# lks1248/SPH-EXA

Hardware: AMD Instinct MI355X
Metric: particle-updates/sec (whole node), Sedov -n 400, 1/2/4/8 MI355X + HBM roofline % (higher is better)
Workload: dtype f32 hydro / f64 coordinates (sph::SphTypes)

## Files before the change

sph-exa_amd/csrc/sx_sim.hpp:

```cpp
#pragma once

#include <hip/hip_runtime.h>

#include <cmath>
#include <initializer_list>
#include <string>
#include <utility>
#include <vector>

#include "../../include/sphexa_hip.h"
#include "sx_comm.hpp"
#include "sx_hydro.hpp"
#include "sx_map.hpp"
#include "sx_profile.hpp"
#include "sx_fof.hpp"
#include "sx_twopoint.hpp"
#include "sx_spectrum.hpp"
#include "sx_step_timer.hpp"
#include "sx_tree.hpp"

namespace sx::turb
{
struct SimTurb;
}
// ... 61 lines not shown
    int      cleanSinceBuild{0};
    uint64_t plainSteps{0};
    uint64_t builds{0}, reuseSteps{0}, staleClusters{0}, exactClusters{0};
    uint64_t resyncs{0};
    uint32_t lastStale{0}, lastExact{0};
    uint64_t stepClusters{0}, stepS13{0};
    bool      xmFused{false};
    uint32_t* exactList{nullptr};
    bool      listsKept{false};
    const void *keptNloc{nullptr}, *keptUni{nullptr}, *keptMask{nullptr}, *keptSame{nullptr}, *keptFrz{nullptr},
        *keptNlocB{nullptr};
    uint64_t  keptClusters{0}, frozenClusters{0};
    uint64_t  earlyExact{0};
    sx::ListsB lb{};
};


struct SkinBuffers
{
    float *   dx{nullptr}, *dy{nullptr}, *dz{nullptr};
    uint32_t* cells{nullptr};
    float *   rel{nullptr}, *hb{nullptr}, *acc{nullptr};
    uint32_t *sloc{nullptr}, *scnt{nullptr}, *ucountS{nullptr}, *l1{nullptr}, *l2{nullptr}, *l3{nullptr};
    uint32_t* host{nullptr};
    uint8_t * streak{nullptr}, *same{nullptr};
    uint32_t* hitmask{nullptr};
    float2*   frz{nullptr};
    uint32_t *nlocB{nullptr}, *ucountB{nullptr}, *hitmaskB{nullptr};
    double *drift{nullptr}, *relg{nullptr}, *x0{nullptr}, *y0{nullptr}, *z0{nullptr};
    float* h0{nullptr};
};

struct ReqBox;

struct DomBuffers
{
    uint32_t* bins{nullptr};
    uint64_t *split{nullptr}, *seg{nullptr}, *cnth{nullptr};
    uint32_t *agree{nullptr}, *agreeh{nullptr};
    unsigned *hflag{nullptr}, *hflagh{nullptr};
    uint32_t* errh{nullptr};
    ReqBox*   mybox{nullptr};
};

struct GravBuffers
{
// ... 135 lines not shown
```

sph-exa_amd/csrc/sx_sim_skin.cpp:

```cpp
#include "sx_sim_internal.hpp"

using namespace sx;
using namespace sx::sim;

namespace
{

__global__ void coverListKernel(const uint32_t* list, uint32_t maxList, uint32_t first, uint32_t last, const double* x,
                                const double* y, const double* z, const float* r, float scale, const ReqBox* boxes,
                                DevBox box, double qmargin, const double* drift, const double* x0, const double* y0,
                                const double* z0, const double* relg, unsigned* flag)
{
    const uint32_t k = blockIdx.x;
    if (k >= min(list[0], maxList)) return;
    const uint32_t i = first + list[1 + k] * kCluster + threadIdx.x;
    if (i >= last) return;
    const ReqBox& b  = boxes[(i - first) / kChunk];
    const double  R  = 2.0 * (double)r[i] * (double)scale * (1.0 + 1e-6) + qmargin;
    const double  Ra = R + drift[0], Rr = R + relg[i];
    const bool    outNow = fabs(foldPbc(x[i] - b.c[0], box, 0)) + Ra > b.s[0] ||
                        fabs(foldPbc(y[i] - b.c[1], box, 1)) + Ra > b.s[1] ||
                        fabs(foldPbc(z[i] - b.c[2], box, 2)) + Ra > b.s[2];
    const bool    outBuild = fabs(foldPbc(x0[i] - b.c[0], box, 0)) + Rr > b.s[0] ||
                          fabs(foldPbc(y0[i] - b.c[1], box, 1)) + Rr > b.s[1] ||
// ... 113 lines not shown
    const bool   ok = skinReserveDisp(s);
    const auto&  B  = s->skinBuf;
    q.dispX = B.dx, q.dispY = B.dy, q.dispZ = B.dz, q.cells = B.cells;
    q.grid  = skinGrid(s->dbox);
    if (!ok) return false;
    return hipMemsetAsync(q.cells, 0xff, 3 * nc * sizeof(uint32_t), st) == hipSuccess &&
           hipMemsetAsync(q.cells + 3 * nc, 0, 3 * nc * sizeof(uint32_t), st) == hipSuccess;
}

static bool skinReserveSearch(sx_sim* s, const NsArgs& na, uint32_t ncl, bool twoSets)
{
    auto&      B    = s->skinBuf;
    auto&      M    = s->mem;
    const bool disp = skinReserveDisp(s);
    B.rel     = M.get<float>("skin.rel", s->cap);
    B.sloc    = M.get<uint32_t>("skin.sloc", na.numGroups * (size_t)nlocWords(s->skin.ngmaxS) * kWave);
    B.scnt    = M.get<uint32_t>("skin.scnt", s->cap);
    B.hb      = M.get<float>("skin.hb", s->cap);
    B.acc     = M.get<float>("skin.acc", ncl);
    B.ucountS = M.get<uint32_t>("skin.ucount", ncl);
    B.l1      = M.get<uint32_t>("skin.l1", ncl + 1);
    B.l2      = M.get<uint32_t>("skin.l2", ncl + 1);
    B.l3      = M.get<uint32_t>("skin.l3", ncl + 1);
    B.host    = M.pinned<uint32_t>("skin.host", 4);
    B.streak  = M.get<uint8_t>("skin.streak", ncl);
    B.hitmask = M.get<uint32_t>("skin.hitmask", na.numGroups * (size_t)kSkinMaskWords * kWave);
    B.same    = M.get<uint8_t>("skin.same", ncl);
    B.frz     = M.get<float2>("skin.frz", ncl);
    B.nlocB    = twoSets ? M.get<uint32_t>("skin.nlocB", na.numGroups * (size_t)nlocWords(na.ngmax) * kWave) : nullptr;
    B.ucountB  = twoSets ? M.get<uint32_t>("skin.ucountB", ncl) : nullptr;
    B.hitmaskB = twoSets ? M.get<uint32_t>("skin.hitmaskB", na.numGroups * (size_t)kSkinMaskWords * kWave) : nullptr;
    return disp && B.rel && B.sloc && B.scnt && B.hb && B.acc && B.ucountS && B.l1 && B.l2 && B.l3 && B.host &&
           B.streak && B.hitmask && B.same && B.frz && (!twoSets || (B.nlocB && B.ucountB && B.hitmaskB));
}

int skinSearch(sx_sim* s, const NsArgs& na, bool reuse, hipStream_t st, float* xmOut, RecT* rtXm, SkinCounts& out)
{
    auto&          K   = s->skin;
    const uint32_t ncl = (na.numGroups + kClusterWaves - 1) / kClusterWaves;
    out                = SkinCounts{};
    out.clusters       = ncl;
    if (!reuse) K.built = K.cur;
    if (!ncl) return SX_OK;
    if (!reuse) K.ngmaxS = skinCapacity(s->p.ngmax, K.built);
    const bool twoSets = na.ucap / 4 >= (uint32_t)kSkinCap && !getenv("SX_SKIN_ONESET");
    if (!skinReserveSearch(s, na, ncl, twoSets)) return SX_ERR_NOMEM;
    const SkinBuffers& B = s->skinBuf;
    uint32_t *const l1 = B.l1, *const l2 = B.l2, *const l3 = B.l3, *const hl = B.host;
    uint32_t* const hmask = B.hitmask, *const nlocB = B.nlocB;
    uint8_t* const  same  = B.same;
    float2* const   frz   = B.frz;

    const SkinGrid g = skinGrid(s->dbox);
    SkinArgs fa{};
    fa.first = na.first, fa.last = na.last, fa.numGroups = na.numGroups, fa.ngmax = na.ngmax, fa.ng0 = na.ng0;
// ... 20 lines not shown
    b.skin1    = 1.0f + K.built;
    b.iterateH = 0;
    b.nloc     = B.sloc;
    b.packMax  = 0;
    b.ngmax    = K.ngmaxS;
    b.nc       = B.scnt;
    b.rxOut    = nullptr;
    b.uoff     = uoff;
    b.ucount   = B.ucountS;

    SIM_HIP(hipMemsetAsync(l1, 0, 4, st));
    SIM_HIP(hipMemsetAsync(l2, 0, 4, st));
    if (!reuse)
    {
        SIM_HIP(hipMemsetAsync(B.streak, 0, ncl, st));
        SIM_HIP(findNeighbors(b, st));
        fa.fresh = 1;
    }
    else fa.fresh = 0;
    fa.list  = nullptr;
    fa.stale = l1;
    fa.streak = reuse ? B.streak : nullptr;
    fa.direct = reuse ? l2 : nullptr;
    SIM_HIP(skinFilter(fa, ncl, st));
    SIM_HIP(hipMemcpyAsync(hl, l1, 4, hipMemcpyDeviceToHost, st));
    SIM_HIP(hipMemcpyAsync(hl + 1, l2, 4, hipMemcpyDeviceToHost, st));
    SIM_HIP(hipStreamSynchronize(st));
    const uint32_t n1 = hl[0], nd = hl[1];
    uint32_t       n2 = nd;
    out.rebuilt = n1, out.stale = n1 + nd, out.exact = nd;
    NsArgs         x  = na;
    NsPolicy large;
    large.mode = 1;
    if (reuse) b.policy = x.policy = &large;
    if ((n1 || nd) && reuse)
    {
        double* c3 = s->mem.get<double>("skin.centers", 3 * (size_t)s->tree.numNodes);
        double* s3 = s->mem.get<double>("skin.sizes", 3 * (size_t)s->tree.numNodes);
        if (!c3 || !s3) return SX_ERR_NOMEM;
        SIM_HIP(skinRefreshBoxes(s->tree, na.x, na.y, na.z, na.box, c3, s3, st));
        b.centers = x.centers = c3;
        b.sizes = x.sizes = s3;
    }
    const bool early = n1 && nd && reuse && s->auxStream && s->evAuxIn && s->evAuxOut && !getenv("SX_SKIN_SERIAL_EXACT");
    if (early)
    {
// ... 6 lines not shown
        if (!sh || atoi(sh) != 0)
        {
            const unsigned G = searchGrid();
            xd.maxGrid       = std::min(nd, G / 2);
            b.maxGrid        = G - xd.maxGrid;
        }
        if (!xd.work || !xd.hSave || !xd.hitMasks) return SX_ERR_NOMEM;
        SIM_HIP(hipEventRecord(s->evAuxIn, st));
        SIM_HIP(hipStreamWaitEvent(s->auxStream, s->evAuxIn, 0));
        SIM_HIP(findNeighbors(xd, s->auxStream));
        SIM_HIP(hipEventRecord(s->evAuxOut, s->auxStream));
    }
    uint32_t* lx = l2;
    if (n1)
    {
        b.subset  = l1;
        SIM_HIP(findNeighbors(b, st));
        fa.fresh  = 1;
        fa.list   = l1;
        if (early) SIM_HIP(hipMemsetAsync(l3, 0, 4, st));
        fa.stale  = early ? l3 : l2;
        fa.streak = nullptr;
        fa.direct = nullptr;
        SIM_HIP(skinFilter(fa, ncl, st));
        SIM_HIP(hipMemcpyAsync(hl + 2, fa.stale, 4, hipMemcpyDeviceToHost, st));
        SIM_HIP(hipStreamSynchronize(st));
        n2 = hl[2];
    }
    uint32_t n3 = 0;
    if (early)
    {
        n3 = n2, n2 = nd + n3, lx = l3;
        K.earlyExact += nd;
        SIM_HIP(hipStreamWaitEvent(st, s->evAuxOut, 0));
    }
    out.exact = n2;
    {
        if (early ? n3 : n2)
        {
            x.subset = lx;
            SIM_HIP(findNeighbors(x, st));
        }
        if (early)
        {
            if (n3) SIM_HIP(hipMemcpyAsync(l2 + 1 + nd, l3 + 1, 4 * (size_t)n3, hipMemcpyDeviceToDevice, st));
            hl[3] = n2;
// ... 121 lines not shown
```

sph-exa_amd/csrc/sx_skin.hip:

```cpp
#include "sx_kernel_poly.hpp"
#include "sx_skin.hpp"
#include "sx_traverse.hpp"

namespace sx
{

namespace
{

constexpr int kWalkPF  = 8;
constexpr int kWalkBlocks = (nlocWords(256) + kWalkPF - 1) / kWalkPF;
constexpr int kB       = kCluster;

__device__ __forceinline__ int cellIndex(double v, const SkinGrid& g, int d) { return gridCell(v, g, d); }

__device__ __forceinline__ float keepOrZero(float v, bool k)
{
    return __builtin_bit_cast(float, __builtin_bit_cast(uint32_t, v) & (0u - (uint32_t)k));
}

__device__ __forceinline__ float norm3up(float x, float y, float z)
{
    return sqrtf(fmaf(x, x, fmaf(y, y, z * z))) * (1.0f + 0x1p-18f) + 1e-30f;
}
// ... 95 lines not shown
    {
        for (int k = 1; k < (int)(blockDim.x >> 6); ++k)
            mx = max(mx, s_max[0][k]), mu = max(mu, s_max[1][k]), kp += s_max[2][k], fz += s_max[3][k], st += s_sum[0][k],
            te += s_sum[1][k], un += s_sum[2][k];
        stats[2]                                          = mx;
        stats[18]                                         = kp;
        stats[19]                                         = fz;
        stats[12]                                         = mu;
        *reinterpret_cast<unsigned long long*>(stats + 4) = st;
        *reinterpret_cast<unsigned long long*>(stats + 6) = te;
        *reinterpret_cast<unsigned long long*>(stats + 8) = un;
    }
}

__device__ __forceinline__ void pushStale(const SkinArgs& a, uint32_t c)
{
    uint32_t* L = (a.direct && a.streak && a.streak[c]) ? a.direct : a.stale;
    L[1 + atomicAdd(&L[0], 1u)] = c;
    if (a.streak) a.streak[c] = 1;
    if (a.same) a.same[c] = 0;
}
static_assert((kWalkBlocks + 1) / 2 <= (int)kSkinMaskWords, "hit-mask words per target");

__global__ __launch_bounds__(kB) __attribute__((amdgpu_waves_per_eu(4))) void skinFilterKernel(SkinArgs a,
                                                                                              uint32_t numClusters)
{
    __shared__ float4   s_rec[kSkinCap];
    __shared__ uint8_t  s_hit[kSkinCap + 4];
    __shared__ uint16_t s_bm[kWalkBlocks][kB];
    uint16_t* const     s_rank = reinterpret_cast<uint16_t*>(s_rec);
    __shared__ float    s_red[kClusterWaves];
    __shared__ int      s_vote[kClusterWaves];
    __shared__ uint32_t s_wsum[kClusterWaves];
    __shared__ uint4    s_cst[kClusterWaves];

    const uint32_t nWork = a.list ? __builtin_amdgcn_readfirstlane(a.list[0]) : numClusters;
    if (blockIdx.x >= nWork) return;
    const uint32_t blk  = a.list ? blockIdx.x : xcdBlock(blockIdx.x, gridDim.x);
    const uint32_t c    = __builtin_amdgcn_readfirstlane(a.list ? a.list[1 + blk] : blk);
    const int      wave = __builtin_amdgcn_readfirstlane(threadIdx.x >> 6), lane = threadIdx.x & 63;
    const uint32_t gw   = c * kClusterWaves + wave;
    const uint32_t c0   = a.first + c * kCluster;
    const uint32_t i    = c0 + threadIdx.x;
    const bool     valid = gw < a.numGroups && i < a.last;
    const uint32_t iS    = valid ? i : c0;
    const double   xi = a.x[iS], yi = a.y[iS], zi = a.z[iS];
    const double   ox = a.x[c0], oy = a.y[c0], oz = a.z[c0];
    float          hi   = a.h[iS];
    const float    h0   = hi;
    const float    hbi  = a.fresh ? hi : a.hb[iS];
    const float    ux = a.dispX[c0], uy = a.dispY[c0], uz = a.dispZ[c0];
    const float    di = a.fresh ? 0.0f
                                : a.rel[iS] + norm3up(a.dispX[iS] - ux, a.dispY[iS] - uy, a.dispZ[iS] - uz);
    const float    Ri = 2.0f * (hbi * a.skin1);
    const uint32_t scount = valid ? a.scnt[i] - 1u : 0u;
    const uint32_t U      = __builtin_amdgcn_readfirstlane(a.ucountS[c]);
    const float    kEps   = 0x1p-16f;
    const uint32_t lstate    = (a.same && a.keepLists && !a.fresh) ? (uint32_t)a.same[c] : 0u;
    const uint32_t lcur      = (a.nlocB && (lstate & kListsBSel)) ? 1u : 0u;
    const bool     curValid  = ((lstate >> lcur) & 1u) != 0;
    const bool     mayFreeze = a.frz && curValid;
    const float2   fref      = mayFreeze ? a.frz[c] : make_float2(-INFINITY, -INFINITY);
    auto           blockBits = [&](uint32_t v) -> uint32_t {
        uint32_t w = 0;
#pragma unroll
        for (int k = 0; k < 3; ++k)
            w |= __ballot((v >> k) & 1u) != 0 ? 1u << k : 0u;
        if (lane == 0) s_vote[wave] = (int)w;
        __syncthreads();
        uint32_t any = 0;
        for (int k = 0; k < kClusterWaves; ++k)
            any |= (uint32_t)s_vote[k];
        __syncthreads();
        return any;
    };
    auto blockAny = [&](bool v) -> bool { return blockBits(v ? 1u : 0u) != 0; };

    float A = 0.0f;
    if (!a.fresh)
    {
        const double rx = foldPbc(xi - ox, a.box, 0), ry = foldPbc(yi - oy, a.box, 1), rz = foldPbc(zi - oz, a.box, 2);
        double       lo[3]  = {valid ? rx : INFINITY, valid ? ry : INFINITY, valid ? rz : INFINITY};
        double       hb3[3] = {valid ? rx : -INFINITY, valid ? ry : -INFINITY, valid ? rz : -INFINITY};
        float        rmax   = valid ? Ri : 0.0f;
        for (int d = 0; d < 3; ++d)
        {
            lo[d]  = -waveMax(-lo[d]);
            hb3[d] = waveMax(hb3[d]);
        }
        rmax      = waveMax(rmax);
        float gmx = 0.0f;
        if (rmax > 0.0f)
        {
            const double o[3] = {ox, oy, oz};
            int          k0[3], nk[3];
            uint32_t     total = 1;
            for (int d = 0; d < 3; ++d)
            {
                k0[d]  = cellIndex(o[d] + lo[d] - (double)rmax, a.grid, d);
                int k1 = cellIndex(o[d] + hb3[d] + (double)rmax, a.grid, d);
                nk[d]  = k1 - k0[d] + 1;
                if (a.grid.pbc[d] && nk[d] >= a.grid.n) k0[d] = 0, nk[d] = a.grid.n;
                total *= nk[d];
            }
            for (uint32_t q = lane; q < total; q += kWave)
            {
                int      k[3];
                uint32_t r = q;
                for (int d = 0; d < 3; ++d)
                {
                    const uint32_t rq = r / (uint32_t)nk[d];
                    k[d]              = k0[d] + (int)(r - rq * (uint32_t)nk[d]);
                    r                 = rq;
                    if (a.grid.pbc[d]) k[d] = wrapCell(k[d], a.grid.n);
                }
                const size_t nc   = (size_t)a.grid.n * a.grid.n * a.grid.n;
                const size_t cell = ((size_t)k[2] * a.grid.n + k[1]) * a.grid.n + k[0];
                const uint32_t lx = a.cells[cell], ly = a.cells[nc + cell], lz = a.cells[2 * nc + cell];
                if (lx != 0xffffffffu)
                {
                    const float ex = fmaxf(fabsf(orderedFloat(lx) - ux), fabsf(orderedFloat(a.cells[3 * nc + cell]) - ux));
                    const float ey = fmaxf(fabsf(orderedFloat(ly) - uy), fabsf(orderedFloat(a.cells[4 * nc + cell]) - uy));
                    const float ez = fmaxf(fabsf(orderedFloat(lz) - uz), fabsf(orderedFloat(a.cells[5 * nc + cell]) - uz));
                    gmx = fmaxf(gmx, norm3up(ex, ey, ez));
                }
            }
        }
        gmx = waveMax(gmx);
        if (lane == 0) s_red[wave] = gmx;
        __syncthreads();
        float g = s_red[0];
        for (int w = 1; w < kClusterWaves; ++w)
            g = fmaxf(g, s_red[w]);
        A = a.acc[c] + g;
        __syncthreads();
    }
    auto withinSkin = [&](float h) { return 2.0f * h + di + A <= Ri * (1.0f - kEps); };
    bool frozen = false;
    {
        const bool bad  = valid && (scount > a.ngmaxS || !withinSkin(hi));
        const bool thin = !a.fresh && valid && 2.0f * hi + 2.0f * (di + A) > Ri * (1.0f - kEps);
        const float e    = di + A + kEps * Ri;
        const bool  melt = valid && !(e + 2.0f * hi < fref.x && e - 2.0f * hi < fref.y);
        const uint32_t v = blockBits((bad ? 1u : 0u) | (thin ? 2u : 0u) | (melt ? 4u : 0u));
        if ((v & 1u) || U > (uint32_t)kSkinCap || U > a.ucap - a.uoff)
        {
            if (threadIdx.x == 0) pushStale(a, c);
            return;
        }
        if ((v & 2u) && threadIdx.x == 0) atomicAdd(&a.stats[13], 1u);
        frozen = mayFreeze && !(v & 4u);
    }
    int      iteration = 0;
    unsigned count = 0, stored = 0;
    const float mi   = a.m[iS];
    float    rho0    = mi;
    bool     kept    = frozen;
    uint32_t ue      = 0;
    float    frzK    = -INFINITY;
    const float xr = (float)foldPbc(xi - ox, a.box, 0), yr = (float)foldPbc(yi - oy, a.box, 1),
                zr = (float)foldPbc(zi - oz, a.box, 2);
    auto setLists = [&](uint32_t k) { return (k ? a.nlocB : a.nloc) + (size_t)gw * nlocWords(a.ngmax) * kWave + lane; };
    auto setUnion = [&](uint32_t k) { return a.uni + (size_t)c * a.ucap + (k ? a.uoffB : 0u); };
    auto setCount = [&](uint32_t k) { return k ? a.ucountB + c : a.ucount + c; };
    auto setMask  = [&](uint32_t k) {
        uint32_t* m = k ? a.hitMaskB : a.hitMask;
        return m ? m + (size_t)gw * kSkinMaskWords * kWave + lane : nullptr;
    };
    const uint32_t* const ll = setLists(lcur);
    auto stage = [&](const uint32_t* list, uint32_t n) -> float {
        constexpr int S = (kSkinCap + kB - 1) / kB;
        uint32_t      js[S];
#pragma unroll
        for (int q = 0; q < S; ++q)
        {
            js[q] = list[min(threadIdx.x + q * kB, n ? n - 1u : 0u)];
        }
        double px[S], py[S], pz[S];
        float  mq[S];
#pragma unroll
        for (int q = 0; q < S; ++q)
            px[q] = a.x[js[q]], py[q] = a.y[js[q]], pz[q] = a.z[js[q]], mq[q] = a.m[js[q]];
        float pm = 0.0f;
#pragma unroll
        for (int q = 0; q < S; ++q)
        {
            const uint32_t u = threadIdx.x + q * kB;
            if (u < n)
            {
                const float fx = (float)foldPbc(px[q] - ox, a.box, 0);
                const float fy = (float)foldPbc(py[q] - oy, a.box, 1);
                const float fz = (float)foldPbc(pz[q] - oz, a.box, 2);
                s_rec[u]       = make_float4(fx, fy, fz, mq[q]);
                pm             = fmaxf(pm, fabsf(fx) + fabsf(fy) + fabsf(fz));
            }
        }
        pm = waveMax(pm);
        if (lane == 0) s_red[wave] = pm;
        __syncthreads();
        float r = s_red[0];
        for (int w = 1; w < kClusterWaves; ++w)
            r = fmaxf(r, s_red[w]);
        return r;
    };

    if (frozen)
    {
        ue = __builtin_amdgcn_readfirstlane(*setCount(lcur));
        (void)stage(setUnion(lcur), ue);
        count  = valid ? a.nc[i] - 1u : 0u;
        stored = min(count, a.ngmax);
        if (a.xmOut && valid && ue <= a.packMax)
        {
            const float     hInv = 1.0f / hi, hInv2 = hInv * hInv;
            const uint32_t  ngr = p12::groups(stored), lastG = ngr ? ngr - 1 : 0u;
            const uint32_t* lp  = ll + (p12::kWords - 1) * lane;
            constexpr int   PW  = 2 * p12::kWords;
            auto            lw  = [&](uint32_t g0, int u) {
                return lp[(size_t)min(g0 + u / p12::kWords, lastG) * (p12::kWords * kWave) + u % p12::kWords];
            };
            uint32_t nx[PW];
#pragma unroll
            for (int u = 0; u < PW; ++u)
                nx[u] = lw(0, u);
            for (uint32_t g0 = 0; g0 < ngr; g0 += 2)
            {
                uint32_t cw[PW];
#pragma unroll
                for (int u = 0; u < PW; ++u)
                {
                    cw[u] = nx[u];
                    nx[u] = lw(g0 + 2, u);
                }
#pragma unroll
                for (int h2 = 0; h2 < 2; ++h2)
                {
                    const uint32_t w0 = cw[3 * h2], w1 = cw[3 * h2 + 1], w2 = cw[3 * h2 + 2];
                    const uint32_t pos[8] = {p12::get<0>(w0, w1, w2), p12::get<1>(w0, w1, w2), p12::get<2>(w0, w1, w2),
                                             p12::get<3>(w0, w1, w2), p12::get<4>(w0, w1, w2), p12::get<5>(w0, w1, w2),
                                             p12::get<6>(w0, w1, w2), p12::get<7>(w0, w1, w2)};
#pragma unroll
                    for (uint32_t e = 0; e < 8; ++e)
                    {
                        const float4 q  = s_rec[min(pos[e], (uint32_t)kSkinCap - 1u)];
                        const float  dx = q.x - xr, dy = q.y - yr, dz = q.z - zr;
                        const float  r2 = fmaf(dx, dx, fmaf(dy, dy, dz * dz));
                        rho0 += keepOrZero(kernelWt(r2 * hInv2) * q.w, 8 * (g0 + h2) + e < stored);
                    }
                }
            }
        }
        else if (a.xmOut && valid)
        {
            const float    hInv = 1.0f / hi, hInv2 = hInv * hInv;
            const uint32_t nw = (stored + 1) >> 1, last = nw ? nw - 1 : 0u;
            constexpr int  PF = kWalkPF;
            uint32_t       nx[PF];
#pragma unroll
            for (int u = 0; u < PF; ++u)
                nx[u] = ll[(size_t)min((uint32_t)u, last) * kWave];
            for (uint32_t w0 = 0; w0 < nw; w0 += PF)
            {
                uint32_t cw[PF];
#pragma unroll
                for (int u = 0; u < PF; ++u)
                {
                    cw[u] = nx[u];
                    nx[u] = ll[(size_t)min(w0 + PF + u, last) * kWave];
                }
#pragma unroll
                for (int u = 0; u < PF; ++u)
                {
                    const uint32_t w = w0 + u;
#pragma unroll
                    for (int h2 = 0; h2 < 2; ++h2)
                    {
                        const float4 q  = s_rec[min(h2 ? cw[u] >> 16 : cw[u] & 0xffffu, (uint32_t)kSkinCap - 1u)];
                        const float  dx = q.x - xr, dy = q.y - yr, dz = q.z - zr;
                        const float  r2 = fmaf(dx, dx, fmaf(dy, dy, dz * dz));
                        rho0 += keepOrZero(kernelWt(r2 * hInv2) * q.w, 2 * w + h2 < stored);
                    }
                }
            }
        }
    }
    else
    {

    const uint32_t* un   = a.uni + (size_t)c * a.ucap + a.uoff;
    const float     pmax = stage(un, U);

    const uint32_t  WS = nlocWords(a.ngmaxS);
    const uint32_t* sl = a.sloc + (size_t)gw * WS * kWave + lane;
    const unsigned  ngmin     = a.ng0 / 4;
    bool            active    = valid;
    auto walk = [&](auto&& begin, auto&& visit, auto&& end) {
        if (!valid) return;
        const uint32_t nw   = (scount + 1) >> 1;
        const uint32_t last = nw ? nw - 1 : 0u;
        constexpr int  PF   = kWalkPF;
        uint32_t       nx[PF];
#pragma unroll
        for (int u = 0; u < PF; ++u)
            nx[u] = sl[(size_t)min((uint32_t)u, last) * kWave];
        for (uint32_t w0 = 0, b = 0; w0 < nw; w0 += PF, ++b)
        {
            uint32_t cw[PF];
#pragma unroll
            for (int u = 0; u < PF; ++u)
            {
// ... 212 lines not shown
    }
    else if (!kept)
    {
        uint32_t* const lw = setLists(ltgt);
        unsigned st = 0;
        uint32_t pend = 0, bits = 0;
        walk([&](uint32_t b) { bits = s_bm[b][threadIdx.x]; },
             [&](uint32_t p, int e, bool) {
                 const bool     keep = ((bits >> e) & 1u) != 0;
                 const uint32_t r    = s_rank[p];
                 const bool     odd  = (st & 1u) != 0;
                 if (keep && odd) lw[(size_t)(st >> 1) * kWave] = pend | (r << 16);
                 pend = (keep && !odd) ? r : pend;
                 st += keep ? 1u : 0u;
             },
             [](uint32_t) {});
        if (st & 1u) lw[(size_t)(st >> 1) * kWave] = pend;
        if (uint32_t* const hm = setMask(ltgt))
            for (uint32_t k = 0; 2 * k < nbl; ++k)
                hm[(size_t)k * kWave] = maskWord(k);
        if (threadIdx.x == 0) *setCount(ltgt) = ue;
    }
    if (threadIdx.x == 0 && a.same && lnew != lstate) a.same[c] = (uint8_t)lnew;
    }

    if (valid)
    {
        if (!frozen)
        {
            a.nc[i] = count + 1;
        }
        if (a.iterateH && iteration > 0) a.h[i] = hi;
        if (a.rxOut) a.rxOut[i] = RecX{xi, yi, zi, hi, a.m[i]};
        if (a.fresh) a.hb[i] = h0;
        a.rel[i] = di;
        if (a.xmOut)
        {
            const float hInv  = 1.0f / hi;
            const float h3Inv = hInv * hInv * hInv;
            const float xm    = (float)((double)mi / ((double)rho0 * a.K * (double)h3Inv));
            a.xmOut[i]        = xm;
            if (a.rtXm) a.rtXm[i] = RecT{xm, 0.0f, 0.0f, 0.0f};
        }
    }
    if (threadIdx.x == 0)
    {
        a.acc[c]    = a.fresh ? 0.0f : A;
        if (a.streak && !a.fresh) a.streak[c] = 0;
    }
    const unsigned           failed = (valid && a.iterateH && iteration >= 10) ? 1u : 0u;
    const unsigned           nfail  = waveSum(failed);
    const unsigned           maxCnt = waveMax(valid ? count : 0u);
    const unsigned long long nst    = waveSum((unsigned long long)(valid ? stored : 0u));
    const unsigned long long walked = waveSum((unsigned long long)scount);
    const float kp = waveMin(valid ? frzK + 2.0f * hi : INFINITY), km = waveMin(valid ? frzK - 2.0f * hi : INFINITY);
    if (lane == 0)
    {
        if (nfail) atomicAdd(&a.stats[1], nfail);
        s_cst[wave]  = make_uint4(maxCnt, (uint32_t)nst, (uint32_t)walked, __float_as_uint(kp));
        s_wsum[wave] = __float_as_uint(km);
    }
    __syncthreads();
    if (threadIdx.x == 0)
    {
        if (a.frz && !frozen)
        {
            float2 f = make_float2(__uint_as_float(s_cst[0].w), __uint_as_float(s_wsum[0]));
            for (int w = 1; w < kClusterWaves; ++w)
                f.x = fminf(f.x, __uint_as_float(s_cst[w].w)), f.y = fminf(f.y, __uint_as_float(s_wsum[w]));
            a.frz[c] = f;
        }
        uint4 t = s_cst[0];
        for (int w = 1; w < kClusterWaves; ++w)
            t.x = max(t.x, s_cst[w].x), t.y += s_cst[w].y, t.z += s_cst[w].z;
        t.y |= (kept ? 0x80000000u : 0u) | (frozen ? 0x40000000u : 0u);
        t.w          = ue;
        a.clStats[c] = t;
    }
}

inline unsigned grid1(size_t n, int b = 256) { return (unsigned)((n + b - 1) / b); }

}

hipError_t skinFilter(const SkinArgs& a, uint32_t numClusters, hipStream_t s)
{
    if (numClusters) skinFilterKernel<<<numClusters, kB, 0, s>>>(a, numClusters);
    return hipGetLastError();
}

hipError_t skinRefreshBoxes(const DevTree& t, const double* x, const double* y, const double* z, const DevBox& box,
                            double* centers, double* sizes, hipStream_t s, bool withCells)
{
    if (t.numNodes <= 0) return hipSuccess;
    leafBoxKernel<<<grid1(t.numNodes, 16), 256, 0, s>>>(t.childOffsets, t.internalToLeaf, t.layout, t.numNodes,
                                                          t.centers, t.sizes, x, y, z, box, centers, sizes,
                                                          withCells ? 1 : 0);
    for (int level = kMaxLevel; level >= 0; --level)
    {
        const int b = t.levelRangeHost[level], e = t.levelRangeHost[level + 1];
        if (e > b) innerBoxKernel<<<grid1(e - b), 256, 0, s>>>(t.childOffsets, b, e, t.centers, box, centers, sizes);
    }
    return hipGetLastError();
}

// ... 14 lines not shown
```

sph-exa_amd/csrc/sx_skin.hpp:

```cpp
#pragma once

#include "sx_tree.hpp"

namespace sx
{

using SkinGrid = DispGrid;

constexpr int kSkinGridN = 64;
constexpr int kSkinCap   = 1920;
constexpr uint32_t kSkinMaskWords = 8;

struct SkinArgs
{
    uint32_t first, last, numGroups, ngmax, ng0;
    uint32_t ngmaxS;
    int      iterateH;
    int      fresh;
    float    skin1;
    const double *x, *y, *z;
    float*       h;
    const float* m;
    uint32_t*    nc;
    RecX*        rxOut;
    uint32_t*       nloc;
    uint32_t        packMax;
    uint32_t*       uni;
    uint32_t*       ucount;
    uint32_t        ucap;
    uint32_t        uoff;
    const uint32_t* ucountS;
    const uint32_t* sloc;
    const uint32_t* scnt;
    float*          hb;
    float*          rel;
    const float *   dispX, *dispY, *dispZ;
    float*          acc;
    const uint32_t* cells;
    SkinGrid        grid;
    const uint32_t* list;
    uint32_t*       stale;
    uint8_t*        streak;
    uint32_t*       direct;
    uint32_t*       hitMask;
    uint8_t*        same;
    int             keepLists;
    uint32_t*       nlocB;
    uint32_t*       ucountB;
    uint32_t*       hitMaskB;
    uint32_t        uoffB;
    float2*         frz;
    DevBox          box;
    const float*    powTab;
    float*          xmOut;
    RecT*           rtXm;
    double          K;
    uint32_t*       stats;
    uint4*          clStats;
};

hipError_t skinFilter(const SkinArgs& a, uint32_t numClusters, hipStream_t s);
hipError_t skinRefreshBoxes(const DevTree& t, const double* x, const double* y, const double* z, const DevBox& box,
                            double* centers, double* sizes, hipStream_t s, bool withCells = false);
hipError_t skinMarkStale(const uint32_t* list, uint32_t numClusters, float* acc, hipStream_t s);
hipError_t reduceClusterStats(const uint4* clStats, uint32_t numClusters, uint32_t* stats, hipStream_t s);

}
```

Baseline: 1.141 billion.

## Split skin filter into decide, frozen-cluster and walk kernels

The monolithic skin filter kernel is split into three kernels. A decide kernel computes the drift bound and classifies each cluster as stale, frozen or walk. A lean frozen kernel with smaller shared staging and higher occupancy recomputes density for frozen clusters. The filter kernel then handles only walk clusters. This is meant to keep the heavy walk path's register and LDS footprint from limiting the common frozen case, at the cost of two extra launches and redundant reads of positions and decision bytes.

```diff
diff --git a/sph-exa_amd/csrc/sx_sim.hpp b/sph-exa_amd/csrc/sx_sim.hpp
--- a/sph-exa_amd/csrc/sx_sim.hpp
+++ b/sph-exa_amd/csrc/sx_sim.hpp
@@ -107,6 +107,7 @@
     uint32_t* cells{nullptr};
     float *   rel{nullptr}, *hb{nullptr}, *acc{nullptr};
     uint32_t *sloc{nullptr}, *scnt{nullptr}, *ucountS{nullptr}, *l1{nullptr}, *l2{nullptr}, *l3{nullptr};
+    uint8_t*  dec{nullptr};
     uint32_t* host{nullptr};
     uint8_t * streak{nullptr}, *same{nullptr};
     uint32_t* hitmask{nullptr};
diff --git a/sph-exa_amd/csrc/sx_sim_skin.cpp b/sph-exa_amd/csrc/sx_sim_skin.cpp
--- a/sph-exa_amd/csrc/sx_sim_skin.cpp
+++ b/sph-exa_amd/csrc/sx_sim_skin.cpp
@@ -159,6 +159,7 @@
     B.l1      = M.get<uint32_t>("skin.l1", ncl + 1);
     B.l2      = M.get<uint32_t>("skin.l2", ncl + 1);
     B.l3      = M.get<uint32_t>("skin.l3", ncl + 1);
+    B.dec     = M.get<uint8_t>("skin.dec", ncl);
     B.host    = M.pinned<uint32_t>("skin.host", 4);
     B.streak  = M.get<uint8_t>("skin.streak", ncl);
     B.hitmask = M.get<uint32_t>("skin.hitmask", na.numGroups * (size_t)kSkinMaskWords * kWave);
@@ -167,7 +168,7 @@
     B.nlocB    = twoSets ? M.get<uint32_t>("skin.nlocB", na.numGroups * (size_t)nlocWords(na.ngmax) * kWave) : nullptr;
     B.ucountB  = twoSets ? M.get<uint32_t>("skin.ucountB", ncl) : nullptr;
     B.hitmaskB = twoSets ? M.get<uint32_t>("skin.hitmaskB", na.numGroups * (size_t)kSkinMaskWords * kWave) : nullptr;
-    return disp && B.rel && B.sloc && B.scnt && B.hb && B.acc && B.ucountS && B.l1 && B.l2 && B.l3 && B.host &&
+    return disp && B.rel && B.sloc && B.scnt && B.hb && B.acc && B.ucountS && B.l1 && B.l2 && B.l3 && B.dec && B.host &&
            B.streak && B.hitmask && B.same && B.frz && (!twoSets || (B.nlocB && B.ucountB && B.hitmaskB));
 }
 
@@ -234,6 +235,14 @@
     fa.stale = l1;
     fa.streak = reuse ? B.streak : nullptr;
     fa.direct = reuse ? l2 : nullptr;
+    if (reuse)
+    {
+        fa.dec = B.dec;
+        const char* fs = getenv("SX_SKIN_FROZEN_STAGE");
+        fa.frozenStage = fs ? (uint32_t)std::max(0, atoi(fs)) : (uint32_t)kSkinFrozenCap;
+        SIM_HIP(skinDecide(fa, ncl, st));
+        SIM_HIP(skinFrozen(fa, ncl, st));
+    }
     SIM_HIP(skinFilter(fa, ncl, st));
     SIM_HIP(hipMemcpyAsync(hl, l1, 4, hipMemcpyDeviceToHost, st));
     SIM_HIP(hipMemcpyAsync(hl + 1, l2, 4, hipMemcpyDeviceToHost, st));
@@ -286,6 +295,7 @@
         fa.stale  = early ? l3 : l2;
         fa.streak = nullptr;
         fa.direct = nullptr;
+        fa.dec    = nullptr;
         SIM_HIP(skinFilter(fa, ncl, st));
         SIM_HIP(hipMemcpyAsync(hl + 2, fa.stale, 4, hipMemcpyDeviceToHost, st));
         SIM_HIP(hipStreamSynchronize(st));
diff --git a/sph-exa_amd/csrc/sx_skin.hip b/sph-exa_amd/csrc/sx_skin.hip
--- a/sph-exa_amd/csrc/sx_skin.hip
+++ b/sph-exa_amd/csrc/sx_skin.hip
@@ -141,6 +141,299 @@
 }
 static_assert((kWalkBlocks + 1) / 2 <= (int)kSkinMaskWords, "hit-mask words per target");
 
+__device__ __forceinline__ uint32_t listState(const SkinArgs& a, uint32_t c)
+{
+    return (a.same && a.keepLists && !a.fresh) ? (uint32_t)a.same[c] : 0u;
+}
+
+__global__ __launch_bounds__(kB) void skinDecideKernel(SkinArgs a)
+{
+    __shared__ float s_red[kClusterWaves];
+    __shared__ int   s_vote[kClusterWaves];
+
+    const uint32_t c    = blockIdx.x;
+    const int      wave = __builtin_amdgcn_readfirstlane(threadIdx.x >> 6), lane = threadIdx.x & 63;
+    const uint32_t gw   = c * kClusterWaves + wave;
+    const uint32_t c0   = a.first + c * kCluster;
+    const uint32_t i    = c0 + threadIdx.x;
+    const bool     valid = gw < a.numGroups && i < a.last;
+    const uint32_t iS    = valid ? i : c0;
+    const double   xi = a.x[iS], yi = a.y[iS], zi = a.z[iS];
+    const double   ox = a.x[c0], oy = a.y[c0], oz = a.z[c0];
+    const float    hi  = a.h[iS];
+    const float    hbi = a.hb[iS];
+    const float    ux = a.dispX[c0], uy = a.dispY[c0], uz = a.dispZ[c0];
+    const float    di = a.rel[iS] + norm3up(a.dispX[iS] - ux, a.dispY[iS] - uy, a.dispZ[iS] - uz);
+    const float    Ri = 2.0f * (hbi * a.skin1);
+    const uint32_t scount = valid ? a.scnt[i] - 1u : 0u;
+    const uint32_t U      = __builtin_amdgcn_readfirstlane(a.ucountS[c]);
+    const float    kEps   = 0x1p-16f;
+    const uint32_t lstate    = listState(a, c);
+    const uint32_t lcur      = (a.nlocB && (lstate & kListsBSel)) ? 1u : 0u;
+    const bool     mayFreeze = a.frz && ((lstate >> lcur) & 1u) != 0;
+    const float2   fref      = mayFreeze ? a.frz[c] : make_float2(-INFINITY, -INFINITY);
+
+    const double rx = foldPbc(xi - ox, a.box, 0), ry = foldPbc(yi - oy, a.box, 1), rz = foldPbc(zi - oz, a.box, 2);
+    double       lo[3]  = {valid ? rx : INFINITY, valid ? ry : INFINITY, valid ? rz : INFINITY};
+    double       hb3[3] = {valid ? rx : -INFINITY, valid ? ry : -INFINITY, valid ? rz : -INFINITY};
+    float        rmax   = valid ? Ri : 0.0f;
+    for (int d = 0; d < 3; ++d)
+    {
+        lo[d]  = -waveMax(-lo[d]);
+        hb3[d] = waveMax(hb3[d]);
+    }
+    rmax      = waveMax(rmax);
+    float gmx = 0.0f;
+    if (rmax > 0.0f)
+    {
+        const double o[3] = {ox, oy, oz};
+        int          k0[3], nk[3];
+        uint32_t     total = 1;
+        for (int d = 0; d < 3; ++d)
+        {
+            k0[d]  = cellIndex(o[d] + lo[d] - (double)rmax, a.grid, d);
+            int k1 = cellIndex(o[d] + hb3[d] + (double)rmax, a.grid, d);
+            nk[d]  = k1 - k0[d] + 1;
+            if (a.grid.pbc[d] && nk[d] >= a.grid.n) k0[d] = 0, nk[d] = a.grid.n;
+            total *= nk[d];
+        }
+        for (uint32_t q = lane; q < total; q += kWave)
+        {
+            int      k[3];
+            uint32_t r = q;
+            for (int d = 0; d < 3; ++d)
+            {
+                const uint32_t rq = r / (uint32_t)nk[d];
+                k[d]              = k0[d] + (int)(r - rq * (uint32_t)nk[d]);
+                r                 = rq;
+                if (a.grid.pbc[d]) k[d] = wrapCell(k[d], a.grid.n);
+            }
+            const size_t nc   = (size_t)a.grid.n * a.grid.n * a.grid.n;
+            const size_t cell = ((size_t)k[2] * a.grid.n + k[1]) * a.grid.n + k[0];
+            const uint32_t lx = a.cells[cell], ly = a.cells[nc + cell], lz = a.cells[2 * nc + cell];
+            if (lx != 0xffffffffu)
+            {
+                const float ex = fmaxf(fabsf(orderedFloat(lx) - ux), fabsf(orderedFloat(a.cells[3 * nc + cell]) - ux));
+                const float ey = fmaxf(fabsf(orderedFloat(ly) - uy), fabsf(orderedFloat(a.cells[4 * nc + cell]) - uy));
+                const float ez = fmaxf(fabsf(orderedFloat(lz) - uz), fabsf(orderedFloat(a.cells[5 * nc + cell]) - uz));
+                gmx = fmaxf(gmx, norm3up(ex, ey, ez));
+            }
+        }
+    }
+    gmx = waveMax(gmx);
+    if (lane == 0) s_red[wave] = gmx;
+    __syncthreads();
+    float g = s_red[0];
+    for (int w = 1; w < kClusterWaves; ++w)
+        g = fmaxf(g, s_red[w]);
+    const float A = a.acc[c] + g;
+
+    const bool bad = valid && (scount > a.ngmaxS || !(2.0f * hi + di + A <= Ri * (1.0f - kEps)));
+    const bool thin = valid && 2.0f * hi + 2.0f * (di + A) > Ri * (1.0f - kEps);
+    const float e    = di + A + kEps * Ri;
+    const bool  melt = valid && !(e + 2.0f * hi < fref.x && e - 2.0f * hi < fref.y);
+    uint32_t w = 0;
+    w |= __ballot(bad) != 0 ? 1u : 0u;
+    w |= __ballot(thin) != 0 ? 2u : 0u;
+    w |= __ballot(melt) != 0 ? 4u : 0u;
+    if (lane == 0) s_vote[wave] = (int)w;
+    __syncthreads();
+    uint32_t v = 0;
+    for (int k = 0; k < kClusterWaves; ++k)
+        v |= (uint32_t)s_vote[k];
+    if ((v & 1u) || U > (uint32_t)kSkinCap || U > a.ucap - a.uoff)
+    {
+        if (threadIdx.x == 0)
+        {
+            pushStale(a, c);
+            a.dec[c] = kSkinStale;
+        }
+        return;
+    }
+    if (valid) a.rel[i] = di;
+    if (threadIdx.x == 0)
+    {
+        if (v & 2u) atomicAdd(&a.stats[13], 1u);
+        a.acc[c] = A;
+        a.dec[c] = (mayFreeze && !(v & 4u)) ? kSkinFrozen : kSkinWalk;
+    }
+}
+
+__global__ __launch_bounds__(kB) __attribute__((amdgpu_waves_per_eu(6))) void skinFrozenKernel(SkinArgs a)
+{
+    __shared__ float4 s_rec[kSkinFrozenCap];
+    __shared__ uint4  s_cst[kClusterWaves];
+
+    const uint32_t c = xcdBlock(blockIdx.x, gridDim.x);
+    if (a.dec[c] != kSkinFrozen) return;
+    const int      wave = __builtin_amdgcn_readfirstlane(threadIdx.x >> 6), lane = threadIdx.x & 63;
+    const uint32_t gw   = c * kClusterWaves + wave;
+    const uint32_t c0   = a.first + c * kCluster;
+    const uint32_t i    = c0 + threadIdx.x;
+    const bool     valid = gw < a.numGroups && i < a.last;
+    const uint32_t iS    = valid ? i : c0;
+    const double   xi = a.x[iS], yi = a.y[iS], zi = a.z[iS];
+    const double   ox = a.x[c0], oy = a.y[c0], oz = a.z[c0];
+    const float    hi = a.h[iS], mi = a.m[iS];
+    const uint32_t count  = valid ? a.nc[i] - 1u : 0u;
+    const uint32_t stored = min(count, a.ngmax);
+    const uint32_t scount = valid ? a.scnt[i] - 1u : 0u;
+    const bool      setB = a.nlocB && (a.same[c] & kListsBSel);
+    const uint32_t* ll   = (setB ? a.nlocB : a.nloc) + (size_t)gw * nlocWords(a.ngmax) * kWave + lane;
+    const uint32_t* un   = a.uni + (size_t)c * a.ucap + (setB ? a.uoffB : 0u);
+    const uint32_t  ue   = __builtin_amdgcn_readfirstlane(setB ? a.ucountB[c] : a.ucount[c]);
+    float           rho0 = mi;
+    const uint32_t  cap  = min(a.frozenStage, (uint32_t)kSkinFrozenCap);
+    if (a.xmOut)
+    {
+        const float xr = (float)foldPbc(xi - ox, a.box, 0), yr = (float)foldPbc(yi - oy, a.box, 1),
+                    zr = (float)foldPbc(zi - oz, a.box, 2);
+        auto record = [&](uint32_t j) {
+            return make_float4((float)foldPbc(a.x[j] - ox, a.box, 0), (float)foldPbc(a.y[j] - oy, a.box, 1),
+                               (float)foldPbc(a.z[j] - oz, a.box, 2), a.m[j]);
+        };
+        {
+            constexpr int  S = 4;
+            const uint32_t ns = min(ue, cap);
+#pragma unroll 1
+            for (uint32_t u0 = threadIdx.x; u0 < ns; u0 += S * kB)
+            {
+                uint32_t js[S];
+#pragma unroll
+                for (int q = 0; q < S; ++q)
+                    js[q] = un[min(u0 + q * kB, ns - 1u)];
+                double px[S], py[S], pz[S];
+                float  mq[S];
+#pragma unroll
+                for (int q = 0; q < S; ++q)
+                    px[q] = a.x[js[q]], py[q] = a.y[js[q]], pz[q] = a.z[js[q]], mq[q] = a.m[js[q]];
+#pragma unroll
+                for (int q = 0; q < S; ++q)
+                    if (u0 + q * kB < ns)
+                        s_rec[u0 + q * kB] = make_float4((float)foldPbc(px[q] - ox, a.box, 0), (float)foldPbc(py[q] - oy, a.box, 1),
+                                                         (float)foldPbc(pz[q] - oz, a.box, 2), mq[q]);
+            }
+            __syncthreads();
+        }
+        const float hInv = 1.0f / hi, hInv2 = hInv * hInv;
+        auto term = [&](uint32_t p, bool k) {
+            const float4 q  = s_rec[min(p, (uint32_t)kSkinFrozenCap - 1u)];
+            const float  dx = q.x - xr, dy = q.y - yr, dz = q.z - zr;
+            const float  r2 = fmaf(dx, dx, fmaf(dy, dy, dz * dz));
+            rho0 += keepOrZero(kernelWt(r2 * hInv2) * q.w, k);
+        };
+        const bool staged = ue <= cap;
+        if (valid && staged && ue <= a.packMax)
+        {
+            const uint32_t  ngr = p12::groups(stored), lastG = ngr ? ngr - 1 : 0u;
+            const uint32_t* lp  = ll + (p12::kWords - 1) * lane;
+            constexpr int   PW  = 2 * p12::kWords;
+            auto            lw  = [&](uint32_t g0, int u) {
+                return lp[(size_t)min(g0 + u / p12::kWords, lastG) * (p12::kWords * kWave) + u % p12::kWords];
+            };
+            uint32_t nx[PW];
+#pragma unroll
+            for (int u = 0; u < PW; ++u)
+                nx[u] = lw(0, u);
+            for (uint32_t g0 = 0; g0 < ngr; g0 += 2)
+            {
+                uint32_t cw[PW];
+#pragma unroll
+                for (int u = 0; u < PW; ++u)
+                {
+                    cw[u] = nx[u];
+                    nx[u] = lw(g0 + 2, u);
+                }
+#pragma unroll
+                for (int h2 = 0; h2 < 2; ++h2)
+                {
+                    const uint32_t w0 = cw[3 * h2], w1 = cw[3 * h2 + 1], w2 = cw[3 * h2 + 2];
+                    const uint32_t pos[8] = {p12::get<0>(w0, w1, w2), p12::get<1>(w0, w1, w2), p12::get<2>(w0, w1, w2),
+                                             p12::get<3>(w0, w1, w2), p12::get<4>(w0, w1, w2), p12::get<5>(w0, w1, w2),
+                                             p12::get<6>(w0, w1, w2), p12::get<7>(w0, w1, w2)};
+#pragma unroll
+                    for (uint32_t e = 0; e < 8; ++e)
+                        term(pos[e], 8 * (g0 + h2) + e < stored);
+                }
+            }
+        }
+        else if (valid && staged)
+        {
+            const uint32_t nw = (stored + 1) >> 1, last = nw ? nw - 1 : 0u;
+            constexpr int  PF = kWalkPF;
+            uint32_t       nx[PF];
+#pragma unroll
+            for (int u = 0; u < PF; ++u)
+                nx[u] = ll[(size_t)min((uint32_t)u, last) * kWave];
+            for (uint32_t w0 = 0; w0 < nw; w0 += PF)
+            {
+                uint32_t cw[PF];
+#pragma unroll
+                for (int u = 0; u < PF; ++u)
+                {
+                    cw[u] = nx[u];
+                    nx[u] = ll[(size_t)min(w0 + PF + u, last) * kWave];
+                }
+#pragma unroll
+                for (int u = 0; u < PF; ++u)
+                {
+                    term(cw[u] & 0xffffu, 2 * (w0 + u) < stored);
+                    term(cw[u] >> 16, 2 * (w0 + u) + 1 < stored);
+                }
+            }
+        }
+        else if (valid)
+        {
+#pragma unroll 1
+            for (uint32_t e = 0; e < stored; ++e)
+            {
+                uint32_t p;
+                if (ue <= a.packMax)
+                {
+                    const uint32_t* g = ll + (p12::kWords - 1) * lane + (size_t)(e / p12::kGroup) * (p12::kWords * kWave);
+                    const uint32_t  w[p12::kWords] = {g[0], g[1], g[2]};
+                    p                              = p12::get(w, e % p12::kGroup);
+                }
+                else
+                {
+                    const uint32_t w = ll[(size_t)(e >> 1) * kWave];
+                    p                = (e & 1u) ? w >> 16 : w & 0xffffu;
+                }
+                const float4 q  = p < cap ? s_rec[p] : record(un[min(p, ue - 1u)]);
+                const float  dx = q.x - xr, dy = q.y - yr, dz = q.z - zr;
+                const float  r2 = fmaf(dx, dx, fmaf(dy, dy, dz * dz));
+                rho0 += kernelWt(r2 * hInv2) * q.w;
+            }
+        }
+    }
+
+    if (valid)
+    {
+        if (a.rxOut) a.rxOut[i] = RecX{xi, yi, zi, hi, mi};
+        if (a.xmOut)
+        {
+            const float hInv  = 1.0f / hi;
+            const float h3Inv = hInv * hInv * hInv;
+            const float xm    = (float)((double)mi / ((double)rho0 * a.K * (double)h3Inv));
+            a.xmOut[i]        = xm;
+            if (a.rtXm) a.rtXm[i] = RecT{xm, 0.0f, 0.0f, 0.0f};
+        }
+    }
+    const uint32_t maxCnt = waveMax(count), nst = waveSum(stored), walked = waveSum(scount);
+    if (lane == 0) s_cst[wave] = make_uint4(maxCnt, nst, walked, 0u);
+    __syncthreads();
+    if (threadIdx.x == 0)
+    {
+        uint4 t = s_cst[0];
+        for (int w = 1; w < kClusterWaves; ++w)
+            t.x = max(t.x, s_cst[w].x), t.y += s_cst[w].y, t.z += s_cst[w].z;
+        t.y |= 0xc0000000u;
+        t.w          = ue;
+        a.clStats[c] = t;
+        if (a.streak) a.streak[c] = 0;
+    }
+}
+
 __global__ __launch_bounds__(kB) __attribute__((amdgpu_waves_per_eu(4))) void skinFilterKernel(SkinArgs a,
                                                                                               uint32_t numClusters)
 {
@@ -157,6 +450,7 @@
     if (blockIdx.x >= nWork) return;
     const uint32_t blk  = a.list ? blockIdx.x : xcdBlock(blockIdx.x, gridDim.x);
     const uint32_t c    = __builtin_amdgcn_readfirstlane(a.list ? a.list[1 + blk] : blk);
+    if (a.dec && a.dec[c] != kSkinWalk) return;
     const int      wave = __builtin_amdgcn_readfirstlane(threadIdx.x >> 6), lane = threadIdx.x & 63;
     const uint32_t gw   = c * kClusterWaves + wave;
     const uint32_t c0   = a.first + c * kCluster;
@@ -168,113 +462,38 @@
     float          hi   = a.h[iS];
     const float    h0   = hi;
     const float    hbi  = a.fresh ? hi : a.hb[iS];
-    const float    ux = a.dispX[c0], uy = a.dispY[c0], uz = a.dispZ[c0];
-    const float    di = a.fresh ? 0.0f
-                                : a.rel[iS] + norm3up(a.dispX[iS] - ux, a.dispY[iS] - uy, a.dispZ[iS] - uz);
+    const float    di = a.fresh ? 0.0f : a.rel[iS];
+    const float    A  = a.fresh ? 0.0f : a.acc[c];
     const float    Ri = 2.0f * (hbi * a.skin1);
     const uint32_t scount = valid ? a.scnt[i] - 1u : 0u;
     const uint32_t U      = __builtin_amdgcn_readfirstlane(a.ucountS[c]);
     const float    kEps   = 0x1p-16f;
-    const uint32_t lstate    = (a.same && a.keepLists && !a.fresh) ? (uint32_t)a.same[c] : 0u;
-    const uint32_t lcur      = (a.nlocB && (lstate & kListsBSel)) ? 1u : 0u;
-    const bool     curValid  = ((lstate >> lcur) & 1u) != 0;
-    const bool     mayFreeze = a.frz && curValid;
-    const float2   fref      = mayFreeze ? a.frz[c] : make_float2(-INFINITY, -INFINITY);
-    auto           blockBits = [&](uint32_t v) -> uint32_t {
-        uint32_t w = 0;
-#pragma unroll
-        for (int k = 0; k < 3; ++k)
-            w |= __ballot((v >> k) & 1u) != 0 ? 1u << k : 0u;
-        if (lane == 0) s_vote[wave] = (int)w;
+    const uint32_t lstate   = listState(a, c);
+    const uint32_t lcur     = (a.nlocB && (lstate & kListsBSel)) ? 1u : 0u;
+    const bool     curValid = ((lstate >> lcur) & 1u) != 0;
+    auto blockAny = [&](bool v) -> bool {
+        const int w = __ballot(v) != 0;
+        if (lane == 0) s_vote[wave] = w;
         __syncthreads();
-        uint32_t any = 0;
+        int any = 0;
         for (int k = 0; k < kClusterWaves; ++k)
-            any |= (uint32_t)s_vote[k];
+            any |= s_vote[k];
         __syncthreads();
-        return any;
+        return any != 0;
     };
-    auto blockAny = [&](bool v) -> bool { return blockBits(v ? 1u : 0u) != 0; };
-
-    float A = 0.0f;
-    if (!a.fresh)
-    {
-        const double rx = foldPbc(xi - ox, a.box, 0), ry = foldPbc(yi - oy, a.box, 1), rz = foldPbc(zi - oz, a.box, 2);
-        double       lo[3]  = {valid ? rx : INFINITY, valid ? ry : INFINITY, valid ? rz : INFINITY};
-        double       hb3[3] = {valid ? rx : -INFINITY, valid ? ry : -INFINITY, valid ? rz : -INFINITY};
-        float        rmax   = valid ? Ri : 0.0f;
-        for (int d = 0; d < 3; ++d)
-        {
-            lo[d]  = -waveMax(-lo[d]);
-            hb3[d] = waveMax(hb3[d]);
-        }
-        rmax      = waveMax(rmax);
-        float gmx = 0.0f;
-        if (rmax > 0.0f)
-        {
-            const double o[3] = {ox, oy, oz};
-            int          k0[3], nk[3];
-            uint32_t     total = 1;
-            for (int d = 0; d < 3; ++d)
-            {
-                k0[d]  = cellIndex(o[d] + lo[d] - (double)rmax, a.grid, d);
-                int k1 = cellIndex(o[d] + hb3[d] + (double)rmax, a.grid, d);
-                nk[d]  = k1 - k0[d] + 1;
-                if (a.grid.pbc[d] && nk[d] >= a.grid.n) k0[d] = 0, nk[d] = a.grid.n;
-                total *= nk[d];
-            }
-            for (uint32_t q = lane; q < total; q += kWave)
-            {
-                int      k[3];
-                uint32_t r = q;
-                for (int d = 0; d < 3; ++d)
-                {
-                    const uint32_t rq = r / (uint32_t)nk[d];
-                    k[d]              = k0[d] + (int)(r - rq * (uint32_t)nk[d]);
-                    r                 = rq;
-                    if (a.grid.pbc[d]) k[d] = wrapCell(k[d], a.grid.n);
-                }
-                const size_t nc   = (size_t)a.grid.n * a.grid.n * a.grid.n;
-                const size_t cell = ((size_t)k[2] * a.grid.n + k[1]) * a.grid.n + k[0];
-                const uint32_t lx = a.cells[cell], ly = a.cells[nc + cell], lz = a.cells[2 * nc + cell];
-                if (lx != 0xffffffffu)
-                {
-                    const float ex = fmaxf(fabsf(orderedFloat(lx) - ux), fabsf(orderedFloat(a.cells[3 * nc + cell]) - ux));
-                    const float ey = fmaxf(fabsf(orderedFloat(ly) - uy), fabsf(orderedFloat(a.cells[4 * nc + cell]) - uy));
-                    const float ez = fmaxf(fabsf(orderedFloat(lz) - uz), fabsf(orderedFloat(a.cells[5 * nc + cell]) - uz));
-                    gmx = fmaxf(gmx, norm3up(ex, ey, ez));
-                }
-            }
-        }
-        gmx = waveMax(gmx);
-        if (lane == 0) s_red[wave] = gmx;
-        __syncthreads();
-        float g = s_red[0];
-        for (int w = 1; w < kClusterWaves; ++w)
-            g = fmaxf(g, s_red[w]);
-        A = a.acc[c] + g;
-        __syncthreads();
-    }
+
     auto withinSkin = [&](float h) { return 2.0f * h + di + A <= Ri * (1.0f - kEps); };
-    bool frozen = false;
-    {
-        const bool bad  = valid && (scount > a.ngmaxS || !withinSkin(hi));
-        const bool thin = !a.fresh && valid && 2.0f * hi + 2.0f * (di + A) > Ri * (1.0f - kEps);
-        const float e    = di + A + kEps * Ri;
-        const bool  melt = valid && !(e + 2.0f * hi < fref.x && e - 2.0f * hi < fref.y);
-        const uint32_t v = blockBits((bad ? 1u : 0u) | (thin ? 2u : 0u) | (melt ? 4u : 0u));
-        if ((v & 1u) || U > (uint32_t)kSkinCap || U > a.ucap - a.uoff)
-        {
-            if (threadIdx.x == 0) pushStale(a, c);
-            return;
-        }
-        if ((v & 2u) && threadIdx.x == 0) atomicAdd(&a.stats[13], 1u);
-        frozen = mayFreeze && !(v & 4u);
+    if (a.fresh && (blockAny(valid && (scount > a.ngmaxS || !withinSkin(hi))) || U > (uint32_t)kSkinCap ||
+                    U > a.ucap - a.uoff))
+    {
+        if (threadIdx.x == 0) pushStale(a, c);
+        return;
     }
     int      iteration = 0;
     unsigned count = 0, stored = 0;
     const float mi   = a.m[iS];
     float    rho0    = mi;
-    bool     kept    = frozen;
+    bool     kept    = false;
     uint32_t ue      = 0;
     float    frzK    = -INFINITY;
     const float xr = (float)foldPbc(xi - ox, a.box, 0), yr = (float)foldPbc(yi - oy, a.box, 1),
@@ -286,7 +505,6 @@
         uint32_t* m = k ? a.hitMaskB : a.hitMask;
         return m ? m + (size_t)gw * kSkinMaskWords * kWave + lane : nullptr;
     };
-    const uint32_t* const ll = setLists(lcur);
     auto stage = [&](const uint32_t* list, uint32_t n) -> float {
         constexpr int S = (kSkinCap + kB - 1) / kB;
         uint32_t      js[S];
@@ -322,89 +540,6 @@
             r = fmaxf(r, s_red[w]);
         return r;
     };
-
-    if (frozen)
-    {
-        ue = __builtin_amdgcn_readfirstlane(*setCount(lcur));
-        (void)stage(setUnion(lcur), ue);
-        count  = valid ? a.nc[i] - 1u : 0u;
-        stored = min(count, a.ngmax);
-        if (a.xmOut && valid && ue <= a.packMax)
-        {
-            const float     hInv = 1.0f / hi, hInv2 = hInv * hInv;
-            const uint32_t  ngr = p12::groups(stored), lastG = ngr ? ngr - 1 : 0u;
-            const uint32_t* lp  = ll + (p12::kWords - 1) * lane;
-            constexpr int   PW  = 2 * p12::kWords;
-            auto            lw  = [&](uint32_t g0, int u) {
-                return lp[(size_t)min(g0 + u / p12::kWords, lastG) * (p12::kWords * kWave) + u % p12::kWords];
-            };
-            uint32_t nx[PW];
-#pragma unroll
-            for (int u = 0; u < PW; ++u)
-                nx[u] = lw(0, u);
-            for (uint32_t g0 = 0; g0 < ngr; g0 += 2)
-            {
-                uint32_t cw[PW];
-#pragma unroll
-                for (int u = 0; u < PW; ++u)
-                {
-                    cw[u] = nx[u];
-                    nx[u] = lw(g0 + 2, u);
-                }
-#pragma unroll
-                for (int h2 = 0; h2 < 2; ++h2)
-                {
-                    const uint32_t w0 = cw[3 * h2], w1 = cw[3 * h2 + 1], w2 = cw[3 * h2 + 2];
-                    const uint32_t pos[8] = {p12::get<0>(w0, w1, w2), p12::get<1>(w0, w1, w2), p12::get<2>(w0, w1, w2),
-                                             p12::get<3>(w0, w1, w2), p12::get<4>(w0, w1, w2), p12::get<5>(w0, w1, w2),
-                                             p12::get<6>(w0, w1, w2), p12::get<7>(w0, w1, w2)};
-#pragma unroll
-                    for (uint32_t e = 0; e < 8; ++e)
-                    {
-                        const float4 q  = s_rec[min(pos[e], (uint32_t)kSkinCap - 1u)];
-                        const float  dx = q.x - xr, dy = q.y - yr, dz = q.z - zr;
-                        const float  r2 = fmaf(dx, dx, fmaf(dy, dy, dz * dz));
-                        rho0 += keepOrZero(kernelWt(r2 * hInv2) * q.w, 8 * (g0 + h2) + e < stored);
-                    }
-                }
-            }
-        }
-        else if (a.xmOut && valid)
-        {
-            const float    hInv = 1.0f / hi, hInv2 = hInv * hInv;
-            const uint32_t nw = (stored + 1) >> 1, last = nw ? nw - 1 : 0u;
-            constexpr int  PF = kWalkPF;
-            uint32_t       nx[PF];
-#pragma unroll
-            for (int u = 0; u < PF; ++u)
-                nx[u] = ll[(size_t)min((uint32_t)u, last) * kWave];
-            for (uint32_t w0 = 0; w0 < nw; w0 += PF)
-            {
-                uint32_t cw[PF];
-#pragma unroll
-                for (int u = 0; u < PF; ++u)
-                {
-                    cw[u] = nx[u];
-                    nx[u] = ll[(size_t)min(w0 + PF + u, last) * kWave];
-                }
-#pragma unroll
-                for (int u = 0; u < PF; ++u)
-                {
-                    const uint32_t w = w0 + u;
-#pragma unroll
-                    for (int h2 = 0; h2 < 2; ++h2)
-                    {
-                        const float4 q  = s_rec[min(h2 ? cw[u] >> 16 : cw[u] & 0xffffu, (uint32_t)kSkinCap - 1u)];
-                        const float  dx = q.x - xr, dy = q.y - yr, dz = q.z - zr;
-                        const float  r2 = fmaf(dx, dx, fmaf(dy, dy, dz * dz));
-                        rho0 += keepOrZero(kernelWt(r2 * hInv2) * q.w, 2 * w + h2 < stored);
-                    }
-                }
-            }
-        }
-    }
-    else
-    {
 
     const uint32_t* un   = a.uni + (size_t)c * a.ucap + a.uoff;
     const float     pmax = stage(un, U);
@@ -663,18 +798,13 @@
         if (threadIdx.x == 0) *setCount(ltgt) = ue;
     }
     if (threadIdx.x == 0 && a.same && lnew != lstate) a.same[c] = (uint8_t)lnew;
-    }
 
     if (valid)
     {
-        if (!frozen)
-        {
-            a.nc[i] = count + 1;
-        }
+        a.nc[i] = count + 1;
         if (a.iterateH && iteration > 0) a.h[i] = hi;
         if (a.rxOut) a.rxOut[i] = RecX{xi, yi, zi, hi, a.m[i]};
-        if (a.fresh) a.hb[i] = h0;
-        a.rel[i] = di;
+        if (a.fresh) a.hb[i] = h0, a.rel[i] = 0.0f;
         if (a.xmOut)
         {
             const float hInv  = 1.0f / hi;
@@ -686,7 +816,7 @@
     }
     if (threadIdx.x == 0)
     {
-        a.acc[c]    = a.fresh ? 0.0f : A;
+        if (a.fresh) a.acc[c] = 0.0f;
         if (a.streak && !a.fresh) a.streak[c] = 0;
     }
     const unsigned           failed = (valid && a.iterateH && iteration >= 10) ? 1u : 0u;
@@ -704,7 +834,7 @@
     __syncthreads();
     if (threadIdx.x == 0)
     {
-        if (a.frz && !frozen)
+        if (a.frz)
         {
             float2 f = make_float2(__uint_as_float(s_cst[0].w), __uint_as_float(s_wsum[0]));
             for (int w = 1; w < kClusterWaves; ++w)
@@ -714,7 +844,7 @@
         uint4 t = s_cst[0];
         for (int w = 1; w < kClusterWaves; ++w)
             t.x = max(t.x, s_cst[w].x), t.y += s_cst[w].y, t.z += s_cst[w].z;
-        t.y |= (kept ? 0x80000000u : 0u) | (frozen ? 0x40000000u : 0u);
+        t.y |= kept ? 0x80000000u : 0u;
         t.w          = ue;
         a.clStats[c] = t;
     }
@@ -722,6 +852,18 @@
 
 inline unsigned grid1(size_t n, int b = 256) { return (unsigned)((n + b - 1) / b); }
 
+}
+
+hipError_t skinDecide(const SkinArgs& a, uint32_t numClusters, hipStream_t s)
+{
+    if (numClusters) skinDecideKernel<<<numClusters, kB, 0, s>>>(a);
+    return hipGetLastError();
+}
+
+hipError_t skinFrozen(const SkinArgs& a, uint32_t numClusters, hipStream_t s)
+{
+    if (numClusters) skinFrozenKernel<<<numClusters, kB, 0, s>>>(a);
+    return hipGetLastError();
 }
 
 hipError_t skinFilter(const SkinArgs& a, uint32_t numClusters, hipStream_t s)
diff --git a/sph-exa_amd/csrc/sx_skin.hpp b/sph-exa_amd/csrc/sx_skin.hpp
--- a/sph-exa_amd/csrc/sx_skin.hpp
+++ b/sph-exa_amd/csrc/sx_skin.hpp
@@ -40,6 +40,8 @@
     SkinGrid        grid;
     const uint32_t* list;
     uint32_t*       stale;
+    uint8_t*        dec;
+    uint32_t        frozenStage;
     uint8_t*        streak;
     uint32_t*       direct;
     uint32_t*       hitMask;
@@ -59,6 +61,12 @@
     uint4*          clStats;
 };
 
+constexpr int kSkinFrozenCap = 1664;
+
+constexpr uint8_t kSkinStale = 0, kSkinFrozen = 1, kSkinWalk = 2;
+
+hipError_t skinDecide(const SkinArgs& a, uint32_t numClusters, hipStream_t s);
+hipError_t skinFrozen(const SkinArgs& a, uint32_t numClusters, hipStream_t s);
 hipError_t skinFilter(const SkinArgs& a, uint32_t numClusters, hipStream_t s);
 hipError_t skinRefreshBoxes(const DevTree& t, const double* x, const double* y, const double* z, const DevBox& box,
                             double* centers, double* sizes, hipStream_t s, bool withCells = false);
```

Result: faster. 1.162 billion (median of 6 runs) (+1.9%).
